# lawfuyang/ToyRenderer

Measured on AMD Instinct MI355X. Metric: Gmeshlets/s culled (whole node), 100M meshlets, higher is better.
Workload: dtype f32

## Files before the change

toyrenderer_amd/csrc/k_gpuculling.hip:

```cpp
#include "cull_math.hip.h"
#include "hzb_quad.hip.h"
#include "instance_cache.hip.h"
#include "trhip_internal.h"

using namespace interop;

namespace
{

constexpr uint32_t kBlock = 256;
constexpr uint32_t kWordSubmit = 1u << 30;
constexpr uint32_t kWordLate = 1u << 31;
constexpr uint32_t kGroupMask = (1u << 27) - 1u;

struct InstanceCullArgs
{
    GPUCullingPassConstants k;
    const BasePassInstanceConstants* instances;
    const uint32_t* ids;
    const MeshData* meshData;
    cm::Hzb hzb;
    MeshletAmplificationData* records;
    uint32_t* dispatchArgs;
    uint32_t* lateCount;
    uint32_t* lateIds;
    const uint32_t* indirectArgs;
    InstanceCullCache cache;
    uint32_t numInstances;
    const uint32_t* shardLate;
    uint32_t directThreads;
    uint32_t maxGroups;
    uint32_t argsWords;
    uint32_t* word;
    uint32_t* localOff;
    uint32_t* blockGroups;
    uint64_t* blockLateSubmit;
    uint32_t* bases;
    uint32_t numBlocks;
    uint32_t* tileHist;
    uint32_t* tileTotal;
    uint16_t* tileOf;
    uint2* lodSel;
    uint32_t* permHeader;
    uint4* perm;
    uint32_t permCapacity;
    uint32_t* lateArgsOut;
    unsigned long long* fusedStatus;
    uint32_t* fusedTicket;
};

struct QuadShare { bool stale = false; };
struct EarlyCullNote { InstanceCullArgs a; size_t scanOp; bool fused; trhip_texture_t* quadOwner = nullptr; std::shared_ptr<QuadShare> share; };

__global__ __launch_bounds__(256) void instanceCacheKernel(const BasePassInstanceConstants* instances, uint32_t n,
                                                           const MeshData* meshData, uint32_t numMeshes, InstanceCullCache c)
{
    const uint32_t i = blockIdx.x * 256u + threadIdx.x;
    if (i >= n) return;
    const BasePassInstanceConstants& inst = instances[i];
    const float4 w0 = *reinterpret_cast<const float4*>(inst.m_WorldMatrix.m[0]);
    const float4 w1 = *reinterpret_cast<const float4*>(inst.m_WorldMatrix.m[1]);
    const float4 w2 = *reinterpret_cast<const float4*>(inst.m_WorldMatrix.m[2]);
    const float4 w3 = *reinterpret_cast<const float4*>(inst.m_WorldMatrix.m[3]);
    const uint32_t meshIdx = inst.m_MeshDataIdx;
    float4 sph = make_float4(0.f, 0.f, 0.f, 0.f);
    uint32_t numLODs = 0;
    uint32_t nm[kMaxNumMeshLODs], mb[kMaxNumMeshLODs];
    float err[kMaxNumMeshLODs];
#pragma unroll
    for (uint32_t l = 0; l < kMaxNumMeshLODs; ++l) { nm[l] = 0; mb[l] = 0; err[l] = 0.f; }
    if (meshIdx < numMeshes) {
        const MeshData& mesh = meshData[meshIdx];
        sph = *reinterpret_cast<const float4*>(&mesh.m_BoundingSphere);
        numLODs = mesh.m_NumLODs;
#pragma unroll
        for (uint32_t l = 0; l < kMaxNumMeshLODs; ++l) {
            nm[l] = mesh.m_MeshLODDatas[l].m_NumMeshlets; mb[l] = mesh.m_MeshLODDatas[l].m_MeshletDataBufferIdx; err[l] = mesh.m_MeshLODDatas[l].m_Error;
        }
    }
    instanceCacheWriteTransformPart(c, i, w0, w1, w2, w3, sph);
    const_cast<float4*>(c.localSphere)[i] = sph;
    const_cast<uint32_t*>(c.numLODs)[i] = numLODs;
#pragma unroll
    for (uint32_t l = 0; l < kMaxNumMeshLODs; ++l) {
        const_cast<uint2&>(c.lod(i, l)) = make_uint2(nm[l], mb[l]);
        const_cast<float&>(c.err(i, l)) = err[l];
    }
}

#ifndef TR_TILES_PER_AXIS
#define TR_TILES_PER_AXIS 16
#endif
constexpr uint32_t kTilesPerAxis = TR_TILES_PER_AXIS;
constexpr uint32_t kNumTiles = kTilesPerAxis * kTilesPerAxis;
constexpr uint32_t kPermHeaderWords = 64;
#ifndef TR_MIN_BINNED
#define TR_MIN_BINNED 4096
#endif
constexpr uint32_t kMinBinnedEntries = TR_MIN_BINNED;

__device__ __forceinline__ uint32_t screenTile(cm::F3 cv, float P00, float P11)
{
    const float iz = __builtin_amdgcn_rcpf(cm::max_(cv.z, 1e-6f));
    const float u = cm::fma_(cv.x * iz * P00, 0.5f, 0.5f), v = cm::fma_(cv.y * iz * P11, -0.5f, 0.5f);
    const int tx = min(max((int)(u * (float)kTilesPerAxis), 0), (int)kTilesPerAxis - 1);
    const int ty = min(max((int)(v * (float)kTilesPerAxis), 0), (int)kTilesPerAxis - 1);
    return (uint32_t)ty * kTilesPerAxis + (uint32_t)tx;
}

template <int LATE>
__device__ __forceinline__ uint32_t threadCount(const InstanceCullArgs& a)
{
    if (LATE) {
        uint32_t count = *a.lateCount;
        uint64_t launched = (uint64_t)a.indirectArgs[0] * kNumThreadsPerWave;
        if (a.shardLate) {
            const uint64_t all = (((uint64_t)a.shardLate[1] + 63u) / 64u) * kNumThreadsPerWave;
            launched = all > a.shardLate[0] ? all - a.shardLate[0] : 0u;
        }
        uint32_t n = launched < count ? (uint32_t)launched : count;
        return n < a.k.m_NbInstances ? n : a.k.m_NbInstances;
    }
    return a.directThreads < a.k.m_NbInstances ? a.directThreads : a.k.m_NbInstances;
}

__device__ __forceinline__ uint32_t waveInclusiveScan(uint32_t v, uint32_t lane)
{
#pragma unroll
    for (int d = 1; d < 64; d <<= 1) {
        uint32_t n = __shfl_up(v, d);
        if (lane >= (uint32_t)d) v += n;
    }
    return v;
}

template <int LATE>
__device__ __forceinline__ uint32_t classify(const InstanceCullArgs& a, uint32_t id, uint32_t* tileOut, uint2* lodOut)
{
    const GPUCullingPassConstants& k = a.k;
    const bool doFrustum = (k.m_CullingFlags & kCullingFlagFrustumCullingEnable) != 0;
    const bool doOcclusion = (k.m_CullingFlags & kCullingFlagOcclusionCullingEnable) != 0;

    const uint32_t cid = id < a.numInstances ? id : 0u;
    const float4 ws = a.cache.sphere[cid];
    const float ms = a.cache.maxScale[cid];
    const cm::F3 wc = { ws.x, ws.y, ws.z };
    const float r = ws.w;
    cm::F3 cv = cm::toView(wc, cm::loadM43(k.m_WorldToView));

    if (!LATE && doFrustum &&
        !cm::frustumVisible(cv, r, k.m_Frustum.x, k.m_Frustum.y, k.m_Frustum.z, k.m_Frustum.w))
        return 0;

    if (doOcclusion) {
        if (!LATE) cv = cm::toView(wc, cm::loadM43(k.m_PrevWorldToView));
        if (!cm::occlusionVisible(cv, r, k.m_NearPlane, k.m_P00, k.m_P11, a.hzb))
            return LATE ? 0 : kWordLate;
    }

    const uint32_t numLODs = a.cache.numLODs[cid];
    uint32_t lod = 0;
    if (k.m_ForcedMeshLOD != kInvalidMeshLOD) {
        const uint32_t last = numLODs - 1u;
        lod = k.m_ForcedMeshLOD < last ? k.m_ForcedMeshLOD : last;
    } else {
        const float distance = cm::max_(cm::sqrt_(cm::dot3(cv, cv)) - r, 0.0f);
        const float threshold = distance * k.m_MeshLODTarget / ms;
        const uint32_t n = numLODs < kMaxNumMeshLODs ? numLODs : kMaxNumMeshLODs;
        for (uint32_t i = 1; i < n; ++i)
            if (a.cache.err(cid, i) < threshold) lod = i;
    }
    lod = lod < kMaxNumMeshLODs ? lod : kMaxNumMeshLODs - 1u;
    const uint2 li = a.cache.lod(cid, lod);
    *lodOut = li;
    const uint32_t numMeshlets = li.x;
    const uint32_t groups = (numMeshlets + kNumThreadsPerWave - 1u) / kNumThreadsPerWave;
    *tileOut = screenTile(cv, k.m_P00, k.m_P11);
    return kWordSubmit | (lod << 27) | (groups & kGroupMask);
}

#ifndef TR_BIG_THREADS
#define TR_BIG_THREADS 512
#endif
#ifndef TR_BIG_PER
#define TR_BIG_PER 1
#endif
constexpr uint32_t kBigThreads = TR_BIG_THREADS;
constexpr uint32_t kBigPerThread = TR_BIG_PER;
constexpr uint32_t kScanThreads = 1024;
constexpr uint32_t kBigChunk = kBigThreads * kBigPerThread;
constexpr uint32_t kBigWaves = kBigThreads / 64;
constexpr uint32_t kScanTilesPerGroup = kNumTiles < 16 ? kNumTiles : 16;
constexpr uint32_t kScanTileGroups = kNumTiles / kScanTilesPerGroup;
constexpr uint32_t kScanStripes = kScanThreads / kScanTilesPerGroup;

template <int LATE>
__device__ __forceinline__ uint32_t activeBigBlocks(const InstanceCullArgs& a, uint32_t n)
{
    const uint32_t need = (n + kBigChunk - 1) / kBigChunk;
    return need < a.numBlocks ? need : a.numBlocks;
}

template <int LATE>
__global__ __launch_bounds__(kBigThreads) void instanceClassifyKernel(InstanceCullArgs a)
{
    __shared__ uint32_t s_hist[kNumTiles];
    __shared__ uint32_t s_waveG[kBigWaves], s_waveL[kBigWaves], s_waveS[kBigWaves];
    const uint32_t n = threadCount<LATE>(a);
    if (blockIdx.x >= activeBigBlocks<LATE>(a, n)) return;
    const uint32_t tid = threadIdx.x, lane = tid & 63u, wave = tid >> 6;
    const bool binned = n >= kMinBinnedEntries;
    for (uint32_t i = tid; i < kNumTiles; i += kBigThreads) s_hist[i] = 0;
    uint32_t carryG = 0, carryL = 0, carryS = 0;
    for (uint32_t e = 0; e < kBigPerThread; ++e) {
        __syncthreads();
        const uint32_t t = blockIdx.x * kBigChunk + e * kBigThreads + tid;
        uint32_t word = 0, tile = 0;
        uint2 lodSel = make_uint2(0u, 0u);
        if (t < n) word = classify<LATE>(a, a.ids[t], &tile, &lodSel);
        const uint32_t g = (word & kWordSubmit) ? (word & kGroupMask) : 0u;
        if (g != 0 && binned) {
            atomicAdd(&s_hist[tile], g);
            a.tileOf[t] = (uint16_t)tile;
            a.lodSel[t] = lodSel;
        }
        const uint32_t late = word >> 31;
        const uint32_t submit = (word >> 30) & 1u;
        const uint32_t incG = waveInclusiveScan(g, lane);
        const uint32_t incL = waveInclusiveScan(late, lane);
        const uint32_t cntS = (uint32_t)__popcll(__ballot(submit != 0));
        if (lane == 63) { s_waveG[wave] = incG; s_waveL[wave] = incL; s_waveS[wave] = cntS; }
        __syncthreads();
        uint32_t baseG = 0, baseL = 0, totG = 0, totL = 0, totS = 0;
#pragma unroll
        for (uint32_t w = 0; w < kBigWaves; ++w) {
            if (w < wave) { baseG += s_waveG[w]; baseL += s_waveL[w]; }
            totG += s_waveG[w]; totL += s_waveL[w]; totS += s_waveS[w];
        }
        if (t < n) {
            a.word[t] = word;
            a.localOff[t] = late ? (carryL + baseL + incL - late) : (carryG + baseG + incG - g);
        }
        carryG += totG; carryL += totL; carryS += totS;
    }
    __syncthreads();
    if (binned)
        for (uint32_t i = tid; i < kNumTiles; i += kBigThreads) a.tileHist[(uint64_t)blockIdx.x * kNumTiles + i] = s_hist[i];
    if (tid == 0) {
        a.blockGroups[blockIdx.x] = carryG;
        a.blockLateSubmit[blockIdx.x] = (uint64_t)carryL | ((uint64_t)carryS << 32);
    }
}

constexpr uint32_t kScanStripsPerGroup = kScanThreads / 256u;
template <int LATE>
__global__ __launch_bounds__(kScanThreads) void instanceScanKernel(InstanceCullArgs a, trhip::QuadArgs q, uint32_t stripEnd)
{
    const uint32_t tid = threadIdx.x, lane = tid & 63u, wave = tid >> 6;
    if (!LATE && blockIdx.x > kScanTileGroups) {
        __shared__ float s_t[kScanStripsPerGroup][9][trhip::kQuadStripCols + 1];
        const uint32_t strip = (blockIdx.x - kScanTileGroups - 1u) * kScanStripsPerGroup + (tid >> 8);
        trhip::hzbQuadStrip(q, strip, s_t[tid >> 8], tid & 255u, strip < stripEnd);
        return;
    }
    if (blockIdx.x != 0) {
        __shared__ uint32_t s_stripe[kScanStripes][kScanTilesPerGroup];
        const uint32_t tl = tid % kScanTilesPerGroup, stripe = tid / kScanTilesPerGroup;
        const uint32_t tile = (blockIdx.x - 1u) * kScanTilesPerGroup + tl;
        constexpr uint32_t kMaxPer = 32;
        const uint32_t perCap = (a.numBlocks + kScanStripes - 1) / kScanStripes;
        if (!LATE && perCap <= kMaxPer) {
            uint32_t v[kMaxPer];
            const uint32_t r0 = stripe * perCap;
#pragma unroll
            for (uint32_t r = 0; r < kMaxPer; ++r)
                v[r] = (r < perCap && r0 + r < a.numBlocks) ? a.tileHist[(uint64_t)(r0 + r) * kNumTiles + tile] : 0u;
            const uint32_t n = threadCount<LATE>(a);
            if (n < kMinBinnedEntries) return;
            const uint32_t activeBlocks = activeBigBlocks<LATE>(a, n);
            uint32_t sum = 0;
#pragma unroll
            for (uint32_t r = 0; r < kMaxPer; ++r) { v[r] = r0 + r < activeBlocks ? v[r] : 0u; sum += v[r]; }
            s_stripe[stripe][tl] = sum;
            __syncthreads();
            uint32_t run = 0;
            for (uint32_t sIdx = 0; sIdx < stripe; ++sIdx) run += s_stripe[sIdx][tl];
#pragma unroll
            for (uint32_t r = 0; r < kMaxPer; ++r) {
                if (r < perCap && r0 + r < activeBlocks) a.tileHist[(uint64_t)(r0 + r) * kNumTiles + tile] = run;
                run += v[r];
            }
            if (stripe == kScanStripes - 1u) a.tileTotal[tile] = run;
            return;
        }
        const uint32_t n = threadCount<LATE>(a);
// ... 43 lines not shown
        for (uint32_t w = 0; w < (kScanThreads / 64); ++w) {
            const uint32_t xg = s_wg[flip][w];
            const uint64_t xl = s_wls[flip][w];
            if (w < wave) { preG += xg; preLS += xl; }
            totG += xg; totLS += xl;
        }
        if (i < activeBlocks) {
            a.blockGroups[i] = carryG + preG + incG - g;
            a.blockLateSubmit[i] = carryLS + preLS + incLS - ls;
        }
        carryG += totG; carryLS += totLS;
        flip ^= 1u;
    }
    if (tid == 0) { s_carryG = carryG; s_carryLS = carryLS; }
    __syncthreads();
    if (tid == 0) {
        const uint32_t baseX = argsX0;
        const uint32_t baseLate = late0;
        a.bases[0] = baseX;
        a.bases[1] = baseLate;
        const uint32_t X = baseX + s_carryG;
        a.dispatchArgs[0] = X;
        if ((uint32_t)(s_carryLS >> 32) != 0) {
            a.dispatchArgs[1] = 1;
            a.dispatchArgs[2] = 1;
        }
        if (a.argsWords > 3) a.dispatchArgs[3] = X;
        if (!LATE) {
            const uint32_t late = baseLate + (uint32_t)s_carryLS;
            *a.lateCount = late;
            if (a.lateArgsOut) {
                a.lateArgsOut[0] = (late + 63u) / 64u;
                a.lateArgsOut[1] = 1;
                a.lateArgsOut[2] = 1;
            }
        }
        a.permHeader[0] = (n >= kMinBinnedEntries && baseX == 0 && X < a.maxGroups && X <= a.permCapacity) ? 1u : 0u;
        a.permHeader[1] = X;
    }
}

constexpr uint32_t kEmitStripsPerGroup = kBigThreads / 256u;
template <int LATE>
__global__ __launch_bounds__(kBigThreads) void instanceEmitKernel(InstanceCullArgs a, trhip::QuadArgs q, uint32_t stripBegin)
{
    if (!LATE && blockIdx.x >= a.numBlocks) {
        __shared__ float s_t[kEmitStripsPerGroup][9][trhip::kQuadStripCols + 1];
        const uint32_t strip = stripBegin + (blockIdx.x - a.numBlocks) * kEmitStripsPerGroup + (threadIdx.x >> 8);
        trhip::hzbQuadStrip(q, strip, s_t[threadIdx.x >> 8], threadIdx.x & 255u, strip < q.firstStrip[q.mips]);
        return;
    }
    __shared__ uint32_t s_cursor[kNumTiles];
    __shared__ uint32_t s_wave[kBigWaves];
    const uint32_t n = threadCount<LATE>(a);
    if (blockIdx.x >= activeBigBlocks<LATE>(a, n)) return;
    const uint32_t tid = threadIdx.x, lane = tid & 63u, wave = tid >> 6;
    const bool binned = n >= kMinBinnedEntries;
    if (binned) {
        uint32_t carry = 0;
        for (uint32_t base = 0; base < kNumTiles; base += kBigThreads) {
            const bool inRange = base + tid < kNumTiles;
            const uint32_t tot = inRange ? a.tileTotal[base + tid] : 0u;
            const uint32_t inc = waveInclusiveScan(tot, lane);
            if (lane == 63) s_wave[wave] = inc;
            __syncthreads();
            uint32_t pre = 0, all = 0;
            for (uint32_t w = 0; w < kBigWaves; ++w) { if (w < wave) pre += s_wave[w]; all += s_wave[w]; }
            if (inRange) s_cursor[base + tid] = carry + pre + inc - tot + a.tileHist[(uint64_t)blockIdx.x * kNumTiles + base + tid];
            carry += all;
            __syncthreads();
        }
    }
    const uint32_t baseG = a.bases[0] + a.blockGroups[blockIdx.x];
    const uint32_t baseL = a.bases[1] + (uint32_t)a.blockLateSubmit[blockIdx.x];
    for (uint32_t e = 0; e < kBigPerThread; ++e) {
        const uint32_t t = blockIdx.x * kBigChunk + e * kBigThreads + tid;
        const uint32_t word = t < n ? a.word[t] : 0u;
        if (word & kWordLate) a.lateIds[baseL + a.localOff[t]] = a.ids[t];
        const bool submit = (word & kWordSubmit) != 0 && !(word & kWordLate);
        const uint32_t groups = word & kGroupMask;
        const uint32_t lod = (word >> 27) & 7u;
        const uint32_t off = submit ? baseG + a.localOff[t] : 0u;
        const bool dropped = submit && off + groups >= a.maxGroups;
        if (dropped && groups != 0 && off < a.maxGroups && a.argsWords > 3) a.dispatchArgs[3] = off;
        const bool emitRec = submit && !dropped;
        const uint32_t id = emitRec ? a.ids[t] : 0u;
        if (emitRec) {
            struct __attribute__((packed, aligned(4))) Quad { uint32_t x, y, z, w; };
            uint32_t* dst = reinterpret_cast<uint32_t*>(a.records + off);
            uint32_t i = 0;
            for (; i + 4u <= groups; i += 4u) {
                const uint32_t o = i * kNumThreadsPerWave;
                *reinterpret_cast<Quad*>(dst + 3u * i) = Quad{ id, lod, o, id };
                *reinterpret_cast<Quad*>(dst + 3u * i + 4u) = Quad{ lod, o + kNumThreadsPerWave, id, lod };
                *reinterpret_cast<Quad*>(dst + 3u * i + 8u) = Quad{ o + 2u * kNumThreadsPerWave, id, lod, o + 3u * kNumThreadsPerWave };
            }
            for (; i < groups; ++i) {
                MeshletAmplificationData rec = { id, lod, i * kNumThreadsPerWave };
                a.records[off + i] = rec;
            }
        }
        const bool place = emitRec && groups != 0 && binned;
        uint32_t p = 0, numMeshlets = 0, mbase = 0;
        if (place) {
            p = atomicAdd(&s_cursor[a.tileOf[t]], groups);
            const uint2 li = a.lodSel[t];
            numMeshlets = li.x; mbase = li.y;
        }
        const uint32_t head = place ? (groups < 4u ? groups : 4u) : 0u;
        const uint32_t j = lane & 3u;
#pragma unroll
        for (uint32_t it = 0; it < 4; ++it) {
            const int src = (int)(it * 16u + (lane >> 2));
            const uint32_t sp = __shfl(p, src), soff = __shfl(off, src), sid = __shfl(id, src);
            const uint32_t sbase = __shfl(mbase, src), snm = __shfl(numMeshlets, src), shead = __shfl(head, src);
            if (j < shead) {
                const uint32_t first = j * kNumThreadsPerWave;
                const uint32_t cnt = snm > first ? (snm - first < kNumThreadsPerWave ? snm - first : kNumThreadsPerWave) : 0u;
                if (sp + j < a.permCapacity) a.perm[sp + j] = make_uint4(soff + j, sid, sbase + first, cnt);
            }
        }
        if (place)
            for (uint32_t i = 4; i < groups; ++i) {
                const uint32_t first = i * kNumThreadsPerWave;
                const uint32_t cnt = numMeshlets > first ? (numMeshlets - first < kNumThreadsPerWave ? numMeshlets - first : kNumThreadsPerWave) : 0u;
                if (p + i < a.permCapacity) a.perm[p + i] = make_uint4(off + i, id, mbase + first, cnt);
            }
    }
}


constexpr uint32_t kFusedMaxEntries = 1u << 17;
constexpr uint32_t kFusedMaxTiles = kFusedMaxEntries / kBlock;
constexpr uint32_t kFusedLateMaxTiles = 4096;
constexpr uint32_t kFusedStatusStride = 16;
constexpr unsigned long long kFusedFlag = 1ull << 63, kFusedPoison = 1ull << 60;

template <int LATE>
__global__ __launch_bounds__(kBlock) void instanceFusedKernel(InstanceCullArgs a, trhip::QuadArgs q)
{
    if (!LATE && blockIdx.x >= a.numBlocks) {
        __shared__ float s_t[9][trhip::kQuadStripCols + 1];
        trhip::hzbQuadStrip(q, blockIdx.x - a.numBlocks, s_t);
        return;
    }
    __shared__ uint32_t s_waveG[kBlock / 64], s_waveL[kBlock / 64], s_waveS[kBlock / 64];
    __shared__ unsigned long long s_preG[kBlock / 64], s_preLS[kBlock / 64];
    __shared__ uint32_t s_tile;
    const uint32_t n = threadCount<LATE>(a);
    const uint32_t numTiles = (n + kBlock - 1) / kBlock < a.numBlocks ? (n + kBlock - 1) / kBlock : a.numBlocks;
    const uint32_t tid = threadIdx.x, lane = tid & 63u, wave = tid >> 6;
    const uint32_t baseX = __hip_atomic_load(&a.dispatchArgs[0], __ATOMIC_RELAXED, __HIP_MEMORY_SCOPE_AGENT);
    const uint32_t baseLate = LATE ? 0u : __hip_atomic_load(a.lateCount, __ATOMIC_RELAXED, __HIP_MEMORY_SCOPE_AGENT);
    if (blockIdx.x >= (numTiles ? numTiles : 1u)) return;
    {
        if (tid == 0) s_tile = atomicAdd(a.fusedTicket, 1u);
        __syncthreads();
        const uint32_t tile = s_tile;
        const uint32_t t = tile * kBlock + tid;
        uint32_t word = 0, tileUnused = 0;
        uint2 lodUnused;
        if (t < n) word = classify<LATE>(a, a.ids[t], &tileUnused, &lodUnused);
        const uint32_t g = (word & kWordSubmit) ? (word & kGroupMask) : 0u;
        const uint32_t late = word >> 31;
        const uint32_t submit = (word >> 30) & 1u;
        const uint32_t incG = waveInclusiveScan(g, lane);
        const uint32_t incL = waveInclusiveScan(late, lane);
        const uint32_t cntS = (uint32_t)__popcll(__ballot(submit != 0));
        if (lane == 63) { s_waveG[wave] = incG; s_waveL[wave] = incL; s_waveS[wave] = cntS; }
        __syncthreads();
        uint32_t baseG = 0, baseL = 0, totG = 0, totL = 0, totS = 0;
#pragma unroll
        for (uint32_t w = 0; w < kBlock / 64; ++w) {
            if (w < wave) { baseG += s_waveG[w]; baseL += s_waveL[w]; }
            totG += s_waveG[w]; totL += s_waveL[w]; totS += s_waveS[w];
        }
        const uint32_t localOff = late ? (baseL + incL - late) : (baseG + incG - g);
        unsigned long long* line = a.fusedStatus + (uint64_t)tile * kFusedStatusStride;
        if (tid == 0 && numTiles != 0) {
            __hip_atomic_store(&line[0], kFusedFlag | (unsigned long long)totG, __ATOMIC_RELAXED, __HIP_MEMORY_SCOPE_AGENT);
            __hip_atomic_store(&line[1], kFusedFlag | ((unsigned long long)totS << 32) | (unsigned long long)totL, __ATOMIC_RELAXED, __HIP_MEMORY_SCOPE_AGENT);
        }
        unsigned long long sumG = 0, sumLS = 0;
        for (uint32_t j = tid; j < tile; j += kBlock) {
            const unsigned long long* pl = a.fusedStatus + (uint64_t)j * kFusedStatusStride;
            unsigned long long v0 = 0, v1 = 0;
            uint32_t spins = 0;
            for (;;) {
                v0 = __hip_atomic_load(&pl[0], __ATOMIC_RELAXED, __HIP_MEMORY_SCOPE_AGENT);
                v1 = __hip_atomic_load(&pl[1], __ATOMIC_RELAXED, __HIP_MEMORY_SCOPE_AGENT);
                if ((v0 & v1 & kFusedFlag) != 0ull) { v0 &= ~kFusedFlag; v1 &= ~kFusedFlag; break; }
                if (++spins > (1u << 22)) { v0 = kFusedPoison; v1 = 0; break; }
                __builtin_amdgcn_s_sleep(1);
            }
            sumG += v0; sumLS += v1;
        }
#pragma unroll
        for (int d = 32; d >= 1; d >>= 1) { sumG += __shfl_xor(sumG, d); sumLS += __shfl_xor(sumLS, d); }
        if (lane == 0) { s_preG[wave] = sumG; s_preLS[wave] = sumLS; }
        __syncthreads();
        unsigned long long preG = 0, preLS = 0;
#pragma unroll
        for (uint32_t w = 0; w < kBlock / 64; ++w) { preG += s_preG[w]; preLS += s_preLS[w]; }
        const uint32_t prefixG = (uint32_t)preG, prefixL = (uint32_t)preLS;
        if (t < n) {
            if (word & kWordLate) {
                a.lateIds[baseLate + prefixL + localOff] = a.ids[t];
            } else if (word & kWordSubmit) {
                const uint32_t groups = word & kGroupMask;
                const uint32_t lod = (word >> 27) & 7u;
                const uint32_t off = baseX + prefixG + localOff;
                if (off + groups >= a.maxGroups) {
                    if (groups != 0 && off < a.maxGroups && a.argsWords > 3) a.dispatchArgs[3] = off;
                } else {
                    const uint32_t id = a.ids[t];
                    for (uint32_t i = 0; i < groups; ++i) {
                        MeshletAmplificationData rec = { id, lod, i * kNumThreadsPerWave };
                        a.records[off + i] = rec;
                    }
                }
            }
        }
        if (tid == 0 && (tile == numTiles - 1u || numTiles == 0)) {
            const unsigned long long allG = preG + totG;
            const uint32_t allL = prefixL + totL, allS = (uint32_t)(preLS >> 32) + totS;
            const uint32_t X = (allG >> 40) ? 0xFFFFFFFFu : baseX + (uint32_t)allG;
            a.bases[0] = baseX;
            a.bases[1] = baseLate;
            a.dispatchArgs[0] = X;
            if (allS != 0) { a.dispatchArgs[1] = 1; a.dispatchArgs[2] = 1; }
            if (a.argsWords > 3 && (X < a.maxGroups || baseX >= a.maxGroups)) a.dispatchArgs[3] = X;
            if (!LATE) {
                const uint32_t lateTotal = baseLate + allL;
                *a.lateCount = lateTotal;
                if (a.lateArgsOut) { a.lateArgsOut[0] = (lateTotal + 63u) / 64u; a.lateArgsOut[1] = 1; a.lateArgsOut[2] = 1; }
            }
            a.permHeader[0] = 0u;
            a.permHeader[1] = X;
        }
    }
}

__global__ void buildLateCullIndirectArgsKernel(const uint32_t* count, uint32_t* args)
{
    args[0] = (count[0] + 63u) / 64u;
    args[1] = 1;
    args[2] = 1;
}

__global__ void shardLateInfoKernel(const uint32_t* counts, uint32_t world, uint32_t rank, uint32_t* info)
{
    uint32_t below = 0, all = 0;
    for (uint32_t p = 0; p < world; ++p) {
        const uint32_t c = counts[p];
        if (p < rank) below += c;
        all += c;
    }
    info[0] = below;
    info[1] = all;
}

int fillHzb(const trhip::DispatchCtx& ctx, trhip_texture_t* tex, const Vector2U& dims, bool occlusion, cm::Hzb* out)
{
    memset(out, 0, sizeof *out);
    if (!occlusion) return TRHIP_OK;
    TRHIP_REQUIRE(tex, "%s: occlusion culling enabled but no HZB texture bound", ctx.shaderName);
    TRHIP_REQUIRE(tex->format == TRHIP_FORMAT_R16_FLOAT, "%s: HZB '%s' is not R16_FLOAT", ctx.shaderName, tex->name.c_str());
    TRHIP_REQUIRE(tex->width == dims.x && tex->height == dims.y,
// ... 58 lines not shown
    trhip_buffer_t* lateIds = ctx.buffer(TRHIP_BIND_STRUCTURED_UAV, 3);
    trhip_buffer_t* shardLate = LATE ? ctx.buffer(TRHIP_BIND_STRUCTURED_SRV, 4) : nullptr;
    TRHIP_REQUIRE(!shardLate || shardLate->byteSize >= 8, "%s: shard late info (t4) smaller than 8 bytes", ctx.shaderName);
    TRHIP_REQUIRE(instances && ids && meshData && records && args && lateCount && lateIds,
                  "%s: needs SRVs t0..t2 and UAVs u0..u3 (BasePassRenderers.cpp:351-362)", ctx.shaderName);
    const bool occlusion = (k->m_CullingFlags & kCullingFlagOcclusionCullingEnable) != 0;
    TRHIP_REQUIRE(instances->byteSize % sizeof(BasePassInstanceConstants) == 0, "%s: instance buffer size is not a multiple of 144", ctx.shaderName);
    TRHIP_REQUIRE(meshData->byteSize % sizeof(MeshData) == 0, "%s: mesh data buffer size is not a multiple of 156", ctx.shaderName);
    TRHIP_REQUIRE(records->byteSize >= sizeof(MeshletAmplificationData), "%s: amplification buffer too small", ctx.shaderName);
    TRHIP_REQUIRE(args->byteSize >= 12, "%s: dispatch-arguments buffer smaller than 12 bytes", ctx.shaderName);
    if (LATE) {
        TRHIP_REQUIRE(ctx.indirect, "%s: LATE_CULL=1 is dispatched indirectly (BasePassRenderers.cpp:399)", ctx.shaderName);
        TRHIP_REQUIRE(occlusion, "%s: LATE_CULL=1 without occlusion culling", ctx.shaderName);
        TRHIP_REQUIRE((uint64_t)k->m_NbInstances * 4 <= lateIds->byteSize, "%s: late id buffer smaller than m_NbInstances", ctx.shaderName);
    } else {
        TRHIP_REQUIRE(!ctx.indirect, "%s: LATE_CULL=0 is dispatched directly", ctx.shaderName);
        TRHIP_REQUIRE((uint64_t)k->m_NbInstances * 4 <= ids->byteSize, "%s: m_NbInstances %u exceeds the id buffer", ctx.shaderName, k->m_NbInstances);
        if (occlusion)
            TRHIP_REQUIRE((uint64_t)k->m_NbInstances * 4 <= lateIds->byteSize, "%s: late id buffer smaller than m_NbInstances", ctx.shaderName);
    }
    TRHIP_REQUIRE(lateCount->byteSize >= 4, "%s: late counter buffer too small", ctx.shaderName);

    InstanceCullArgs a;
    memset(&a, 0, sizeof a);
    a.k = *k;
    int rc = fillHzb(ctx, hzb, k->m_HZBDimensions, occlusion, &a.hzb);
    if (rc != TRHIP_OK) return rc;
    a.instances = (const BasePassInstanceConstants*)instances->ptr;
    a.ids = LATE ? (const uint32_t*)lateIds->ptr : (const uint32_t*)ids->ptr;
    a.meshData = (const MeshData*)meshData->ptr;
    a.records = (MeshletAmplificationData*)records->ptr;
    a.dispatchArgs = (uint32_t*)args->ptr;
    a.lateCount = (uint32_t*)lateCount->ptr;
    a.lateIds = (uint32_t*)lateIds->ptr;
    a.indirectArgs = LATE ? (const uint32_t*)((const char*)ctx.argsBuffer->ptr + ctx.argsOffset) : nullptr;
    a.shardLate = shardLate ? (const uint32_t*)shardLate->ptr : nullptr;
    const uint64_t direct = (uint64_t)ctx.gx * kNumThreadsPerWave;
    a.directThreads = direct > 0xFFFFFFFFull ? 0xFFFFFFFFu : (uint32_t)direct;
    const uint64_t cap = records->byteSize / sizeof(MeshletAmplificationData);
    a.maxGroups = cap > 0xFFFFFFFFull ? 0xFFFFFFFFu : (uint32_t)cap;
    a.argsWords = args->byteSize >= 16 ? 4u : 3u;

    const uint32_t nMax = k->m_NbInstances;
    if (nMax == 0) return TRHIP_OK;

    rc = trhip::instanceCacheEnsure(instances);
    if (rc != TRHIP_OK) return rc;
    a.cache = instanceCacheLayout(instances->cullCache.ptr, instances->byteSize / sizeof(BasePassInstanceConstants));
    a.numInstances = (uint32_t)(instances->byteSize / sizeof(BasePassInstanceConstants));
    ctx.emit("instance_cache", [instances, meshData](hipStream_t s) { return trhip::instanceCacheLaunchBuild(instances, meshData, s); });
    static const bool noFused = getenv("TRHIP_NO_FUSED_INSTANCE") != nullptr;
    const bool fusedPath = (nMax <= kFusedMaxEntries || (LATE && (nMax + kBlock - 1) / kBlock <= kFusedLateMaxTiles)) && !noFused;
    a.numBlocks = fusedPath ? (nMax + kBlock - 1) / kBlock : (nMax + kBigChunk - 1) / kBigChunk;
    a.word = (uint32_t*)ctx.scratch((size_t)nMax * 4);
    a.localOff = (uint32_t*)ctx.scratch((size_t)nMax * 4);
    a.blockGroups = (uint32_t*)ctx.scratch((size_t)a.numBlocks * 4);
    a.blockLateSubmit = (uint64_t*)ctx.scratch((size_t)a.numBlocks * 8);
    a.bases = (uint32_t*)ctx.scratch(16);
    a.tileHist = (uint32_t*)ctx.scratch(fusedPath ? 16 : (size_t)a.numBlocks * kNumTiles * 4);
    a.tileTotal = (uint32_t*)ctx.scratch(kNumTiles * 4);
    a.tileOf = (uint16_t*)ctx.scratch((size_t)nMax * 2);
    a.lodSel = (uint2*)ctx.scratch((size_t)nMax * 8);
    TRHIP_REQUIRE(a.word && a.localOff && a.blockGroups && a.blockLateSubmit && a.bases && a.tileHist && a.tileTotal && a.tileOf && a.lodSel, "%s: scratch allocation failed", ctx.shaderName);
    rc = records->order.allocate(records->dev, (uint64_t)kPermHeaderWords * 4 + (uint64_t)a.maxGroups * 16);
    if (rc != TRHIP_OK) return rc;
    a.permHeader = (uint32_t*)records->order.ptr;
    a.perm = (uint4*)(a.permHeader + kPermHeaderWords);
    a.permCapacity = a.maxGroups;
    const bool wantTable = !LATE && occlusion && a.maxGroups >= trhip::tableMinGroups();
    if (wantTable) {
        rc = trhip::hzbQuadEnsure(hzb);
        if (rc != TRHIP_OK) return rc;
    }

    if (fusedPath) {
        const size_t words = (size_t)a.numBlocks * kFusedStatusStride * 2 + 4;
        uint32_t* mem = (uint32_t*)ctx.scratch(words * 4);
        TRHIP_REQUIRE(mem, "%s: scratch allocation failed", ctx.shaderName);
        rc = ctx.cl->recordClearWords(mem, words, 0, true);
        if (rc != TRHIP_OK) return rc;
        a.fusedStatus = (unsigned long long*)mem;
        a.fusedTicket = mem + (size_t)a.numBlocks * kFusedStatusStride * 2;
        trhip_texture_t* quadOwner = wantTable ? hzb : nullptr;
        if (quadOwner) ctx.cl->use(quadOwner->quad.ptr, ctx.cl->ops.size(), true);
        if (LATE) ctx.emit("fused", [a](hipStream_t s) {
            trhip::QuadArgs q;
            memset(&q, 0, sizeof q);
            TRHIP_LAUNCH(instanceFusedKernel<LATE>, dim3(a.numBlocks), dim3(kBlock), 0, s, a, q);
            return trhip::launchStatus("instanceFusedKernel"); });
        else ctx.emit("fused", fusedEarlyLaunch(a, quadOwner));
        if (!LATE && occlusion) ctx.cl->peephole = { ctx.cl->ops.size() - 1, "gpuculling_early", std::make_shared<EarlyCullNote>(EarlyCullNote{ a, ctx.cl->ops.size() - 1, true, quadOwner }) };
        return TRHIP_OK;
    }

    ctx.emit("classify", [a](hipStream_t s) {
        TRHIP_LAUNCH(instanceClassifyKernel<LATE>, dim3(a.numBlocks), dim3(kBigThreads), 0, s, a);
        return trhip::launchStatus("instanceClassifyKernel"); });
    trhip_texture_t* quadOwner = wantTable ? hzb : nullptr;
    std::shared_ptr<QuadShare> share = quadOwner ? std::make_shared<QuadShare>() : nullptr;
    if (quadOwner) ctx.cl->use(quadOwner->quad.ptr, ctx.cl->ops.size(), true);
    if (LATE) ctx.emit("scan", [a](hipStream_t s) {
        trhip::QuadArgs q;
        memset(&q, 0, sizeof q);
        TRHIP_LAUNCH(instanceScanKernel<LATE>, dim3(1 + kScanTileGroups), dim3(kScanThreads), 0, s, a, q, 0u);
        return trhip::launchStatus("instanceScanKernel"); });
    else ctx.emit("scan", scanEarlyLaunch(a, quadOwner, share));
    const size_t scanOp = ctx.cl->ops.size() - 1;
    if (quadOwner) ctx.cl->use(quadOwner->quad.ptr, ctx.cl->ops.size(), true);
    ctx.emit("emit", [a, quadOwner, share](hipStream_t s) {
        trhip::QuadArgs q;
        memset(&q, 0, sizeof q);
        uint32_t extra = 0, stripBegin = 0;
        if (!LATE && quadOwner && share && share->stale) {
            q = trhip::quadArgs(quadOwner);
            stripBegin = quadScanStrips(q.firstStrip[q.mips]);
            extra = (q.firstStrip[q.mips] - stripBegin + kEmitStripsPerGroup - 1u) / kEmitStripsPerGroup;
// ... 75 lines not shown
```

Before: 122.8.

## Pack per-instance classify outputs into one uint4 entry and hoist loads in cull kernels

Replaces the separate word, localOff, tileOf and lodSel scratch arrays with a single 16-byte entry per instance, so the tile sits in the low bits of the word. The scatter kernel then loads everything in one vector load, issued early together with tile totals and histogram rows before the block-level early exit. The classify step is restructured to issue all instance-cache loads (LOD errors, lod0 info, HZB texel pairs) up front and branch-free, with HZB mip offsets parked in shared memory. This trades extra speculative loads and registers for fewer dependent memory round-trips and less divergence. It also adds a new header of inline footprint and projection helpers.

```diff
diff --git a/toyrenderer_amd/csrc/instance_loads.hip.h b/toyrenderer_amd/csrc/instance_loads.hip.h
--- /dev/null
+++ b/toyrenderer_amd/csrc/instance_loads.hip.h
@@ -0,0 +1,90 @@
+#pragma once
+
+#include <stdint.h>
+
+#include <hip/hip_runtime.h>
+
+#include "ShaderInterop.h"
+
+namespace il
+{
+
+__host__ __device__ inline uint32_t clampId(uint32_t id, uint32_t numInstances) { return id < numInstances ? id : 0u; }
+
+__host__ __device__ inline uint64_t lodPlaneIndex(uint32_t cid, uint32_t lod, uint64_t stride)
+{
+    const uint32_t l = lod < interop::kMaxNumMeshLODs ? lod : interop::kMaxNumMeshLODs - 1u;
+    return (uint64_t)l * stride + cid;
+}
+
+__host__ __device__ inline int hzbLevel(float width, float height, uint32_t mips)
+{
+    const float m = __builtin_fmaxf(width, height);
+    if (!(m >= 1.0f)) return 0;
+    uint32_t bits;
+    __builtin_memcpy(&bits, &m, 4);
+    const int e = (int)((bits >> 23) & 0xFFu) - 127;
+    const int last = (int)mips - 1;
+    return e > last ? last : e;
+}
+
+struct Footprint
+{
+    uint32_t i0, i1;
+    bool pair;
+    int mip;
+};
+
+__host__ __device__ inline Footprint footprint(float minx, float miny, float maxx, float maxy, float P00, float P11,
+                                               uint32_t hzbWidth, uint32_t hzbHeight, uint32_t mips, const uint32_t* mipOff)
+{
+    float ax = __builtin_fminf(__builtin_fmaxf(minx * P00, -1.0f), 1.0f);
+    float ay = __builtin_fminf(__builtin_fmaxf(miny * P11, -1.0f), 1.0f);
+    float az = __builtin_fminf(__builtin_fmaxf(maxx * P00, -1.0f), 1.0f);
+    float aw = __builtin_fminf(__builtin_fmaxf(maxy * P11, -1.0f), 1.0f);
+    ax = __builtin_fmaf(ax, 0.5f, 0.5f);
+    ay = __builtin_fmaf(ay, -0.5f, 0.5f);
+    az = __builtin_fmaf(az, 0.5f, 0.5f);
+    aw = __builtin_fmaf(aw, -0.5f, 0.5f);
+    const float width = (az - ax) * (float)hzbWidth;
+    const float height = (aw - ay) * (float)hzbHeight;
+    const int mip = hzbLevel(width, height, mips);
+    const float u = (ax + az) * 0.5f, v = (ay + aw) * 0.5f;
+    const uint32_t mw = (hzbWidth >> mip) ? (hzbWidth >> mip) : 1u;
+    const uint32_t mh = (hzbHeight >> mip) ? (hzbHeight >> mip) : 1u;
+    const float fx = __builtin_fmaf(u, (float)mw, -0.5f);
+    const float fy = __builtin_fmaf(v, (float)mh, -0.5f);
+    const float flx = __builtin_floorf(fx), fly = __builtin_floorf(fy);
+    int x0 = (int)flx, y0 = (int)fly;
+    const bool wx1 = (fx - flx) > 0.0f, wy1 = (fy - fly) > 0.0f;
+    const int xm = (int)mw - 1, ym = (int)mh - 1;
+    int x1 = x0 + 1 < 0 ? 0 : (x0 + 1 > xm ? xm : x0 + 1), y1 = y0 + 1 < 0 ? 0 : (y0 + 1 > ym ? ym : y0 + 1);
+    x0 = x0 < 0 ? 0 : (x0 > xm ? xm : x0);
+    y0 = y0 < 0 ? 0 : (y0 > ym ? ym : y0);
+    x1 = wx1 ? x1 : x0;
+    y1 = wy1 ? y1 : y0;
+    const uint32_t base = mipOff[mip];
+    Footprint f;
+    f.i0 = base + (uint32_t)y0 * mw + (uint32_t)x0;
+    f.i1 = base + (uint32_t)y1 * mw + (uint32_t)x0;
+    f.pair = x1 != x0;
+    f.mip = mip;
+    return f;
+}
+
+struct Quotients { float minx, miny, maxx, maxy; };
+__host__ __device__ inline Quotients projectSphere(float cx, float cy, float cz, float r)
+{
+    const float crx = cx * r, cry = cy * r, crz = cz * r;
+    const float czr2 = __builtin_fmaf(cz, cz, -(r * r));
+    const float vx = __builtin_sqrtf(__builtin_fmaf(cx, cx, czr2));
+    const float vy = __builtin_sqrtf(__builtin_fmaf(cy, cy, czr2));
+    Quotients q;
+    q.minx = __builtin_fmaf(vx, cx, -crz) / __builtin_fmaf(vx, cz, crx);
+    q.maxx = __builtin_fmaf(vx, cx, crz) / __builtin_fmaf(vx, cz, -crx);
+    q.miny = __builtin_fmaf(vy, cy, -crz) / __builtin_fmaf(vy, cz, cry);
+    q.maxy = __builtin_fmaf(vy, cy, crz) / __builtin_fmaf(vy, cz, -cry);
+    return q;
+}
+
+}
diff --git a/toyrenderer_amd/csrc/k_gpuculling.hip b/toyrenderer_amd/csrc/k_gpuculling.hip
--- a/toyrenderer_amd/csrc/k_gpuculling.hip
+++ b/toyrenderer_amd/csrc/k_gpuculling.hip
@@ -1,6 +1,7 @@
 #include "cull_math.hip.h"
 #include "hzb_quad.hip.h"
 #include "instance_cache.hip.h"
+#include "instance_loads.hip.h"
 #include "trhip_internal.h"
 
 using namespace interop;
@@ -31,16 +32,13 @@
     uint32_t directThreads;
     uint32_t maxGroups;
     uint32_t argsWords;
-    uint32_t* word;
-    uint32_t* localOff;
+    uint4* entry;
     uint32_t* blockGroups;
     uint64_t* blockLateSubmit;
     uint32_t* bases;
     uint32_t numBlocks;
     uint32_t* tileHist;
     uint32_t* tileTotal;
-    uint16_t* tileOf;
-    uint2* lodSel;
     uint32_t* permHeader;
     uint4* perm;
     uint32_t permCapacity;
@@ -93,6 +91,7 @@
 #endif
 constexpr uint32_t kTilesPerAxis = TR_TILES_PER_AXIS;
 constexpr uint32_t kNumTiles = kTilesPerAxis * kTilesPerAxis;
+static_assert((kNumTiles & (kNumTiles - 1u)) == 0u && kNumTiles <= kGroupMask + 1u, "the tile shares the entry word with lod / submit / late: masked to kNumTiles - 1");
 constexpr uint32_t kPermHeaderWords = 64;
 #ifndef TR_MIN_BINNED
 #define TR_MIN_BINNED 4096
@@ -134,48 +133,78 @@
     return v;
 }
 
+__device__ __forceinline__ void parkMipOffsets(const cm::Hzb& h, uint32_t* s_mipOff, uint32_t tid)
+{
+    uint32_t v = 0;
+#pragma unroll
+    for (uint32_t i = 0; i < 16; ++i) v = tid == i ? h.mipOffset[i] : v;
+    if (tid < 16) s_mipOff[tid] = v;
+}
+
 template <int LATE>
-__device__ __forceinline__ uint32_t classify(const InstanceCullArgs& a, uint32_t id, uint32_t* tileOut, uint2* lodOut)
+__device__ __forceinline__ uint32_t classify(const InstanceCullArgs& a, uint32_t id, bool valid, const uint32_t* s_mipOff, uint32_t* tileOut, uint2* lodOut)
 {
     const GPUCullingPassConstants& k = a.k;
     const bool doFrustum = (k.m_CullingFlags & kCullingFlagFrustumCullingEnable) != 0;
     const bool doOcclusion = (k.m_CullingFlags & kCullingFlagOcclusionCullingEnable) != 0;
-
-    const uint32_t cid = id < a.numInstances ? id : 0u;
+    const bool forced = k.m_ForcedMeshLOD != kInvalidMeshLOD;
+
+    const uint32_t cid = il::clampId(id, a.numInstances);
     const float4 ws = a.cache.sphere[cid];
     const float ms = a.cache.maxScale[cid];
+    const uint32_t numLODs = a.cache.numLODs[cid];
+    const uint2 lod0 = a.cache.lodInfo[il::lodPlaneIndex(cid, 0u, a.cache.stride)];
     const cm::F3 wc = { ws.x, ws.y, ws.z };
     const float r = ws.w;
     cm::F3 cv = cm::toView(wc, cm::loadM43(k.m_WorldToView));
-
-    if (!LATE && doFrustum &&
-        !cm::frustumVisible(cv, r, k.m_Frustum.x, k.m_Frustum.y, k.m_Frustum.z, k.m_Frustum.w))
-        return 0;
-
+    const bool inFrustum = LATE || !doFrustum ||
+        cm::frustumVisible(cv, r, k.m_Frustum.x, k.m_Frustum.y, k.m_Frustum.z, k.m_Frustum.w);
+    if (doOcclusion && !LATE) cv = cm::toView(wc, cm::loadM43(k.m_PrevWorldToView));
+
+    const uint32_t nErr = numLODs < kMaxNumMeshLODs ? numLODs : kMaxNumMeshLODs;
+    float err[kMaxNumMeshLODs];
+#pragma unroll
+    for (uint32_t i = 1; i < kMaxNumMeshLODs; ++i) err[i] = 0.f;
+    if (!forced) {
+#pragma unroll
+        for (uint32_t i = 1; i < kMaxNumMeshLODs; ++i)
+            if (i < nErr) err[i] = a.cache.error[il::lodPlaneIndex(cid, i, a.cache.stride)];
+    }
+    bool occluded = false;
     if (doOcclusion) {
-        if (!LATE) cv = cm::toView(wc, cm::loadM43(k.m_PrevWorldToView));
-        if (!cm::occlusionVisible(cv, r, k.m_NearPlane, k.m_P00, k.m_P11, a.hzb))
-            return LATE ? 0 : kWordLate;
-    }
-
-    const uint32_t numLODs = a.cache.numLODs[cid];
+        const bool accept = (cv.z - k.m_NearPlane) < r;
+        const il::Quotients q = il::projectSphere(cv.x, cv.y, cv.z, r);
+        const il::Footprint f = il::footprint(q.minx, q.miny, q.maxx, q.maxy, k.m_P00, k.m_P11, a.hzb.width, a.hzb.height, a.hzb.mips, s_mipOff);
+        const bool lookup = valid && inFrustum && !accept;
+        const uint32_t row0 = cm::loadTexelPair(a.hzb.base, lookup ? f.i0 : 0u);
+        const uint32_t row1 = cm::loadTexelPair(a.hzb.base, lookup ? f.i1 : 0u);
+        cm::OccSample o;
+        o.accept = accept; o.i0 = f.i0; o.i1 = f.i1; o.pair = f.pair;
+        o.depthSphere = cm::div_(k.m_NearPlane, cv.z - r);
+        occluded = !cm::occlusionResolve(o, row0, row1);
+    }
+
     uint32_t lod = 0;
-    if (k.m_ForcedMeshLOD != kInvalidMeshLOD) {
+    if (forced) {
         const uint32_t last = numLODs - 1u;
         lod = k.m_ForcedMeshLOD < last ? k.m_ForcedMeshLOD : last;
     } else {
         const float distance = cm::max_(cm::sqrt_(cm::dot3(cv, cv)) - r, 0.0f);
         const float threshold = distance * k.m_MeshLODTarget / ms;
-        const uint32_t n = numLODs < kMaxNumMeshLODs ? numLODs : kMaxNumMeshLODs;
-        for (uint32_t i = 1; i < n; ++i)
-            if (a.cache.err(cid, i) < threshold) lod = i;
+#pragma unroll
+        for (uint32_t i = 1; i < kMaxNumMeshLODs; ++i)
+            if (i < nErr && err[i] < threshold) lod = i;
     }
     lod = lod < kMaxNumMeshLODs ? lod : kMaxNumMeshLODs - 1u;
-    const uint2 li = a.cache.lod(cid, lod);
+    const bool submit = valid && inFrustum && !occluded;
+    uint2 li = lod0;
+    if (submit && lod != 0u) li = a.cache.lodInfo[il::lodPlaneIndex(cid, lod, a.cache.stride)];
     *lodOut = li;
     const uint32_t numMeshlets = li.x;
     const uint32_t groups = (numMeshlets + kNumThreadsPerWave - 1u) / kNumThreadsPerWave;
     *tileOut = screenTile(cv, k.m_P00, k.m_P11);
+    if (!valid || !inFrustum) return 0u;
+    if (occluded) return LATE ? 0u : kWordLate;
     return kWordSubmit | (lod << 27) | (groups & kGroupMask);
 }
 
@@ -206,24 +235,23 @@
 {
     __shared__ uint32_t s_hist[kNumTiles];
     __shared__ uint32_t s_waveG[kBigWaves], s_waveL[kBigWaves], s_waveS[kBigWaves];
+    __shared__ uint32_t s_mipOff[16];
     const uint32_t n = threadCount<LATE>(a);
     if (blockIdx.x >= activeBigBlocks<LATE>(a, n)) return;
     const uint32_t tid = threadIdx.x, lane = tid & 63u, wave = tid >> 6;
     const bool binned = n >= kMinBinnedEntries;
+    parkMipOffsets(a.hzb, s_mipOff, tid);
     for (uint32_t i = tid; i < kNumTiles; i += kBigThreads) s_hist[i] = 0;
     uint32_t carryG = 0, carryL = 0, carryS = 0;
     for (uint32_t e = 0; e < kBigPerThread; ++e) {
+        const uint32_t t = blockIdx.x * kBigChunk + e * kBigThreads + tid;
+        const uint32_t id = t < n ? a.ids[t] : 0u;
         __syncthreads();
-        const uint32_t t = blockIdx.x * kBigChunk + e * kBigThreads + tid;
-        uint32_t word = 0, tile = 0;
+        uint32_t tile = 0;
         uint2 lodSel = make_uint2(0u, 0u);
-        if (t < n) word = classify<LATE>(a, a.ids[t], &tile, &lodSel);
+        const uint32_t word = classify<LATE>(a, id, t < n, s_mipOff, &tile, &lodSel);
         const uint32_t g = (word & kWordSubmit) ? (word & kGroupMask) : 0u;
-        if (g != 0 && binned) {
-            atomicAdd(&s_hist[tile], g);
-            a.tileOf[t] = (uint16_t)tile;
-            a.lodSel[t] = lodSel;
-        }
+        if (g != 0 && binned) atomicAdd(&s_hist[tile], g);
         const uint32_t late = word >> 31;
         const uint32_t submit = (word >> 30) & 1u;
         const uint32_t incG = waveInclusiveScan(g, lane);
@@ -237,10 +265,8 @@
             if (w < wave) { baseG += s_waveG[w]; baseL += s_waveL[w]; }
             totG += s_waveG[w]; totL += s_waveL[w]; totS += s_waveS[w];
         }
-        if (t < n) {
-            a.word[t] = word;
-            a.localOff[t] = late ? (carryL + baseL + incL - late) : (carryG + baseG + incG - g);
-        }
+        if (t < n)
+            a.entry[t] = make_uint4((word & ~kGroupMask) | tile, late ? (carryL + baseL + incL - late) : (carryG + baseG + incG - g), lodSel.x, lodSel.y);
         carryG += totG; carryL += totL; carryS += totS;
     }
     __syncthreads();
@@ -390,39 +416,62 @@
     }
     __shared__ uint32_t s_cursor[kNumTiles];
     __shared__ uint32_t s_wave[kBigWaves];
+    const uint32_t tid = threadIdx.x, lane = tid & 63u, wave = tid >> 6;
+    constexpr uint32_t kTileRounds = (kNumTiles + kBigThreads - 1) / kBigThreads;
+    uint32_t tot[kTileRounds], histRow[kTileRounds];
+#pragma unroll
+    for (uint32_t i = 0; i < kTileRounds; ++i) {
+        const uint32_t tileIdx = i * kBigThreads + tid < kNumTiles ? i * kBigThreads + tid : kNumTiles - 1u;
+        tot[i] = a.tileTotal[tileIdx];
+        histRow[i] = a.tileHist[(uint64_t)blockIdx.x * kNumTiles + tileIdx];
+    }
+    const uint32_t bases0 = a.bases[0], bases1 = a.bases[1];
+    const uint32_t blockG = a.blockGroups[blockIdx.x];
+    const uint32_t blockL = reinterpret_cast<const uint32_t*>(a.blockLateSubmit)[2u * blockIdx.x];
+    uint4 entryIn[kBigPerThread];
+    uint32_t idIn[kBigPerThread];
+#pragma unroll
+    for (uint32_t e = 0; e < kBigPerThread; ++e) {
+        const uint32_t t = blockIdx.x * kBigChunk + e * kBigThreads + tid;
+        const uint32_t tc = t < a.k.m_NbInstances ? t : a.k.m_NbInstances - 1u;
+        entryIn[e] = a.entry[tc];
+        idIn[e] = a.ids[tc];
+    }
     const uint32_t n = threadCount<LATE>(a);
     if (blockIdx.x >= activeBigBlocks<LATE>(a, n)) return;
-    const uint32_t tid = threadIdx.x, lane = tid & 63u, wave = tid >> 6;
     const bool binned = n >= kMinBinnedEntries;
     if (binned) {
         uint32_t carry = 0;
-        for (uint32_t base = 0; base < kNumTiles; base += kBigThreads) {
+#pragma unroll
+        for (uint32_t i = 0; i < kTileRounds; ++i) {
+            const uint32_t base = i * kBigThreads;
             const bool inRange = base + tid < kNumTiles;
-            const uint32_t tot = inRange ? a.tileTotal[base + tid] : 0u;
-            const uint32_t inc = waveInclusiveScan(tot, lane);
+            if (!inRange) tot[i] = 0u;
+            const uint32_t inc = waveInclusiveScan(tot[i], lane);
             if (lane == 63) s_wave[wave] = inc;
             __syncthreads();
             uint32_t pre = 0, all = 0;
             for (uint32_t w = 0; w < kBigWaves; ++w) { if (w < wave) pre += s_wave[w]; all += s_wave[w]; }
-            if (inRange) s_cursor[base + tid] = carry + pre + inc - tot + a.tileHist[(uint64_t)blockIdx.x * kNumTiles + base + tid];
+            if (inRange) s_cursor[base + tid] = carry + pre + inc - tot[i] + histRow[i];
             carry += all;
             __syncthreads();
         }
     }
-    const uint32_t baseG = a.bases[0] + a.blockGroups[blockIdx.x];
-    const uint32_t baseL = a.bases[1] + (uint32_t)a.blockLateSubmit[blockIdx.x];
+    const uint32_t baseG = bases0 + blockG;
+    const uint32_t baseL = bases1 + blockL;
+#pragma unroll
     for (uint32_t e = 0; e < kBigPerThread; ++e) {
         const uint32_t t = blockIdx.x * kBigChunk + e * kBigThreads + tid;
-        const uint32_t word = t < n ? a.word[t] : 0u;
-        if (word & kWordLate) a.lateIds[baseL + a.localOff[t]] = a.ids[t];
+        const uint32_t word = t < n ? entryIn[e].x : 0u;
+        if (word & kWordLate) a.lateIds[baseL + entryIn[e].y] = idIn[e];
         const bool submit = (word & kWordSubmit) != 0 && !(word & kWordLate);
-        const uint32_t groups = word & kGroupMask;
+        const uint32_t groups = submit ? ((entryIn[e].z + kNumThreadsPerWave - 1u) / kNumThreadsPerWave) & kGroupMask : 0u;
         const uint32_t lod = (word >> 27) & 7u;
-        const uint32_t off = submit ? baseG + a.localOff[t] : 0u;
+        const uint32_t off = submit ? baseG + entryIn[e].y : 0u;
         const bool dropped = submit && off + groups >= a.maxGroups;
         if (dropped && groups != 0 && off < a.maxGroups && a.argsWords > 3) a.dispatchArgs[3] = off;
         const bool emitRec = submit && !dropped;
-        const uint32_t id = emitRec ? a.ids[t] : 0u;
+        const uint32_t id = emitRec ? idIn[e] : 0u;
         if (emitRec) {
             struct __attribute__((packed, aligned(4))) Quad { uint32_t x, y, z, w; };
             uint32_t* dst = reinterpret_cast<uint32_t*>(a.records + off);
@@ -441,9 +490,8 @@
         const bool place = emitRec && groups != 0 && binned;
         uint32_t p = 0, numMeshlets = 0, mbase = 0;
         if (place) {
-            p = atomicAdd(&s_cursor[a.tileOf[t]], groups);
-            const uint2 li = a.lodSel[t];
-            numMeshlets = li.x; mbase = li.y;
+            p = atomicAdd(&s_cursor[word & (kNumTiles - 1u)], groups);
+            numMeshlets = entryIn[e].z; mbase = entryIn[e].w;
         }
         const uint32_t head = place ? (groups < 4u ? groups : 4u) : 0u;
         const uint32_t j = lane & 3u;
@@ -485,20 +533,23 @@
     __shared__ uint32_t s_waveG[kBlock / 64], s_waveL[kBlock / 64], s_waveS[kBlock / 64];
     __shared__ unsigned long long s_preG[kBlock / 64], s_preLS[kBlock / 64];
     __shared__ uint32_t s_tile;
-    const uint32_t n = threadCount<LATE>(a);
-    const uint32_t numTiles = (n + kBlock - 1) / kBlock < a.numBlocks ? (n + kBlock - 1) / kBlock : a.numBlocks;
+    __shared__ uint32_t s_mipOff[16];
     const uint32_t tid = threadIdx.x, lane = tid & 63u, wave = tid >> 6;
     const uint32_t baseX = __hip_atomic_load(&a.dispatchArgs[0], __ATOMIC_RELAXED, __HIP_MEMORY_SCOPE_AGENT);
     const uint32_t baseLate = LATE ? 0u : __hip_atomic_load(a.lateCount, __ATOMIC_RELAXED, __HIP_MEMORY_SCOPE_AGENT);
+    const uint32_t n = threadCount<LATE>(a);
+    parkMipOffsets(a.hzb, s_mipOff, tid);
+    const uint32_t numTiles = (n + kBlock - 1) / kBlock < a.numBlocks ? (n + kBlock - 1) / kBlock : a.numBlocks;
     if (blockIdx.x >= (numTiles ? numTiles : 1u)) return;
     {
         if (tid == 0) s_tile = atomicAdd(a.fusedTicket, 1u);
         __syncthreads();
         const uint32_t tile = s_tile;
         const uint32_t t = tile * kBlock + tid;
-        uint32_t word = 0, tileUnused = 0;
+        uint32_t tileUnused = 0;
         uint2 lodUnused;
-        if (t < n) word = classify<LATE>(a, a.ids[t], &tileUnused, &lodUnused);
+        const uint32_t id = t < n ? a.ids[t] : 0u;
+        const uint32_t word = classify<LATE>(a, id, t < n, s_mipOff, &tileUnused, &lodUnused);
         const uint32_t g = (word & kWordSubmit) ? (word & kGroupMask) : 0u;
         const uint32_t late = word >> 31;
         const uint32_t submit = (word >> 30) & 1u;
@@ -543,7 +594,7 @@
         const uint32_t prefixG = (uint32_t)preG, prefixL = (uint32_t)preLS;
         if (t < n) {
             if (word & kWordLate) {
-                a.lateIds[baseLate + prefixL + localOff] = a.ids[t];
+                a.lateIds[baseLate + prefixL + localOff] = id;
             } else if (word & kWordSubmit) {
                 const uint32_t groups = word & kGroupMask;
                 const uint32_t lod = (word >> 27) & 7u;
@@ -551,7 +602,6 @@
                 if (off + groups >= a.maxGroups) {
                     if (groups != 0 && off < a.maxGroups && a.argsWords > 3) a.dispatchArgs[3] = off;
                 } else {
-                    const uint32_t id = a.ids[t];
                     for (uint32_t i = 0; i < groups; ++i) {
                         MeshletAmplificationData rec = { id, lod, i * kNumThreadsPerWave };
                         a.records[off + i] = rec;
@@ -716,16 +766,13 @@
     static const bool noFused = getenv("TRHIP_NO_FUSED_INSTANCE") != nullptr;
     const bool fusedPath = (nMax <= kFusedMaxEntries || (LATE && (nMax + kBlock - 1) / kBlock <= kFusedLateMaxTiles)) && !noFused;
     a.numBlocks = fusedPath ? (nMax + kBlock - 1) / kBlock : (nMax + kBigChunk - 1) / kBigChunk;
-    a.word = (uint32_t*)ctx.scratch((size_t)nMax * 4);
-    a.localOff = (uint32_t*)ctx.scratch((size_t)nMax * 4);
+    a.entry = (uint4*)ctx.scratch(fusedPath ? 16 : (size_t)nMax * 16);
     a.blockGroups = (uint32_t*)ctx.scratch((size_t)a.numBlocks * 4);
     a.blockLateSubmit = (uint64_t*)ctx.scratch((size_t)a.numBlocks * 8);
     a.bases = (uint32_t*)ctx.scratch(16);
     a.tileHist = (uint32_t*)ctx.scratch(fusedPath ? 16 : (size_t)a.numBlocks * kNumTiles * 4);
     a.tileTotal = (uint32_t*)ctx.scratch(kNumTiles * 4);
-    a.tileOf = (uint16_t*)ctx.scratch((size_t)nMax * 2);
-    a.lodSel = (uint2*)ctx.scratch((size_t)nMax * 8);
-    TRHIP_REQUIRE(a.word && a.localOff && a.blockGroups && a.blockLateSubmit && a.bases && a.tileHist && a.tileTotal && a.tileOf && a.lodSel, "%s: scratch allocation failed", ctx.shaderName);
+    TRHIP_REQUIRE(a.entry && a.blockGroups && a.blockLateSubmit && a.bases && a.tileHist && a.tileTotal, "%s: scratch allocation failed", ctx.shaderName);
     rc = records->order.allocate(records->dev, (uint64_t)kPermHeaderWords * 4 + (uint64_t)a.maxGroups * 16);
     if (rc != TRHIP_OK) return rc;
     a.permHeader = (uint32_t*)records->order.ptr;
```

New measurement: 122.6 (median of 3 runs). Within noise of the previous version (-0.2%).
